# dglai/dgl-0.5-benchmark

Measured on AMD Instinct MI355X. Metric: aggregated edges/s, full-graph 3-layer GraphSAGE (hidden 64) on an ogbn-products-shaped graph; epoch time in ms_per_step, higher is better.
Workload: dtype f32

## Files before the change

dgl-0.5-benchmark_amd/csrc/xty.hip:

```cpp
#include "common.h"

namespace mgx {

constexpr int kXtyWaves = 2048;

static int xty_waves(int64_t n) {
  int64_t w = (n / 256 + 63) / 64 * 64;
  if (w < 256) w = 256;
  if (w > kXtyWaves) w = kXtyWaves;
  return (int)w;
}

template <int MT, int KT>
__global__ __launch_bounds__(kBlock) void xty_partial_kernel(int64_t n, int M, int K, const float* __restrict__ A, int64_t lda,
                                                             const float* __restrict__ B, int64_t ldb, float* __restrict__ part) {
  const int lane = threadIdx.x & (kWave - 1);
  const int64_t gw = (int64_t)blockIdx.x * kWavesPerBlock + threadIdx.x / kWave;
  const int c = lane % 16, q = lane / 16;
  v4f acc[MT][KT];
#pragma unroll
  for (int i = 0; i < MT; ++i)
#pragma unroll
    for (int j = 0; j < KT; ++j) acc[i][j] = (v4f)(0.f);
  bool am[MT], bm[KT];
#pragma unroll
  for (int i = 0; i < MT; ++i) am[i] = i * 16 + c < M;
#pragma unroll
// ... 6 lines not shown
      const int64_t row = r0 + s * 4 + q;
      const bool ok = row < n;
#pragma unroll
      for (int i = 0; i < MT; ++i) a[s][i] = (ok && am[i]) ? A[row * lda + i * 16 + c] : 0.f;
#pragma unroll
      for (int j = 0; j < KT; ++j) b[s][j] = (ok && bm[j]) ? B[row * ldb + j * 16 + c] : 0.f;
    }
#pragma unroll
    for (int s = 0; s < 4; ++s)
#pragma unroll
      for (int i = 0; i < MT; ++i)
#pragma unroll
        for (int j = 0; j < KT; ++j) acc[i][j] = __builtin_amdgcn_mfma_f32_16x16x4f32(a[s][i], b[s][j], acc[i][j], 0, 0, 0);
  }
  float* p = part + gw * (int64_t)(MT * 16) * (KT * 16);
#pragma unroll
  for (int i = 0; i < MT; ++i)
#pragma unroll
    for (int j = 0; j < KT; ++j)
#pragma unroll
      for (int r = 0; r < 4; ++r) p[(i * 16 + 4 * q + r) * (KT * 16) + j * 16 + c] = acc[i][j][r];
}

template <int AVG, int AST, int BVG, int BST>
__global__ __launch_bounds__(kBlock) void xty_partial_v4_kernel(int64_t n, int M, int K, int mt16, int kt16, const float* __restrict__ A,
                                                                int64_t lda, const float* __restrict__ B, int64_t ldb,
                                                                float* __restrict__ part, float* __restrict__ part_sum) {
  constexpr int AT = AVG * 4 + AST, BT = BVG * 4 + BST;
  const int lane = threadIdx.x & (kWave - 1);
  const int64_t gw = (int64_t)blockIdx.x * kWavesPerBlock + threadIdx.x / kWave;
  const int c = lane % 16, q = lane / 16;
  v4f acc[AT][BT];
  v4f accs[AT > 0 ? AT : 1];
#pragma unroll
  for (int i = 0; i < AT; ++i) {
    accs[i] = (v4f)(0.f);
#pragma unroll
    for (int j = 0; j < BT; ++j) acc[i][j] = (v4f)(0.f);
  }
  const float one = c == 0 ? 1.f : 0.f;
  const int64_t stride = (int64_t)gridDim.x * kWavesPerBlock * 16;
  for (int64_t r0 = gw * 16; r0 < n; r0 += stride) {
    float a[4][AT > 0 ? AT : 1], b[4][BT > 0 ? BT : 1];
#pragma unroll
    for (int s = 0; s < 4; ++s) {
      const int64_t row = r0 + s * 4 + q;
      const bool ok = row < n;
#pragma unroll
      for (int g = 0; g < AVG; ++g) {
        const v4f v = (ok && g * 64 + 4 * c + 3 < M) ? *reinterpret_cast<const v4f*>(A + row * lda + g * 64 + 4 * c) : (v4f)(0.f);
        a[s][g * 4 + 0] = v.x; a[s][g * 4 + 1] = v.y; a[s][g * 4 + 2] = v.z; a[s][g * 4 + 3] = v.w;
      }
#pragma unroll
      for (int i = 0; i < AST; ++i) a[s][AVG * 4 + i] = (ok && AVG * 64 + i * 16 + c < M) ? A[row * lda + AVG * 64 + i * 16 + c] : 0.f;
#pragma unroll
      for (int g = 0; g < BVG; ++g) {
        const v4f v = (ok && g * 64 + 4 * c + 3 < K) ? *reinterpret_cast<const v4f*>(B + row * ldb + g * 64 + 4 * c) : (v4f)(0.f);
        b[s][g * 4 + 0] = v.x; b[s][g * 4 + 1] = v.y; b[s][g * 4 + 2] = v.z; b[s][g * 4 + 3] = v.w;
      }
#pragma unroll
      for (int j = 0; j < BST; ++j) b[s][BVG * 4 + j] = (ok && BVG * 64 + j * 16 + c < K) ? B[row * ldb + BVG * 64 + j * 16 + c] : 0.f;
    }
#pragma unroll
    for (int s = 0; s < 4; ++s)
#pragma unroll
      for (int i = 0; i < AT; ++i)
#pragma unroll
        for (int j = 0; j < BT; ++j) acc[i][j] = __builtin_amdgcn_mfma_f32_16x16x4f32(a[s][i], b[s][j], acc[i][j], 0, 0, 0);
    if (part_sum) {
#pragma unroll
      for (int s = 0; s < 4; ++s)
#pragma unroll
        for (int i = 0; i < AT; ++i) accs[i] = __builtin_amdgcn_mfma_f32_16x16x4f32(a[s][i], (r0 + s * 4 + q < n) ? one : 0.f, accs[i], 0, 0, 0);
// ... 4 lines not shown
    for (int i = 0; i < AT; ++i)
#pragma unroll
      for (int r = 0; r < 4; ++r) {
        const int mi = 4 * q + r;
        const int m = i < AVG * 4 ? (i / 4) * 64 + 4 * mi + (i % 4) : AVG * 64 + (i - AVG * 4) * 16 + mi;
        if (m < mt16) part_sum[gw * (int64_t)mt16 + m] = accs[i][r];
      }
  }
  float* p = part + gw * (int64_t)mt16 * kt16;
#pragma unroll
  for (int i = 0; i < AT; ++i)
#pragma unroll
    for (int j = 0; j < BT; ++j) {
      const int k = j < BVG * 4 ? (j / 4) * 64 + 4 * c + (j % 4) : BVG * 64 + (j - BVG * 4) * 16 + c;
#pragma unroll
      for (int r = 0; r < 4; ++r) {
        const int mi = 4 * q + r;
        const int m = i < AVG * 4 ? (i / 4) * 64 + 4 * mi + (i % 4) : AVG * 64 + (i - AVG * 4) * 16 + mi;
        if (m < mt16 && k < kt16) p[m * kt16 + k] = acc[i][j][r];
      }
    }
}

template <int AVG, int AST>
static bool launch_xty_v4_b(int bvg, int bst, int waves, int64_t n, int M, int K, int mt16, int kt16, const float* A, int64_t lda,
                            const float* B, int64_t ldb, float* part, float* part_sum, hipStream_t s) {
#define MGX_XTY4(G, T) if (bvg == G && bst == T) { hipLaunchKernelGGL((xty_partial_v4_kernel<AVG, AST, G, T>), dim3(waves / kWavesPerBlock), dim3(kBlock), 0, s, n, M, K, mt16, kt16, A, lda, B, ldb, part, part_sum); return true; }
  MGX_XTY4(2, 0) MGX_XTY4(1, 0) MGX_XTY4(1, 1) MGX_XTY4(1, 2) MGX_XTY4(1, 3) MGX_XTY4(1, 4)
#undef MGX_XTY4
  return false;
}

static bool launch_xty_v4(int mt, int kt, int waves, int64_t n, int M, int K, const float* A, int64_t lda, const float* B, int64_t ldb,
                          float* part, float* part_sum, hipStream_t s) {
  const bool bvec = ldb % 4 == 0 && (uintptr_t)B % 16 == 0 && K % 4 == 0 && K >= 64;
  if (!bvec) return false;
  const int bvg = K >= 128 ? 2 : 1, bst = (K - bvg * 64 + 15) / 16;
  const bool avec = lda % 4 == 0 && (uintptr_t)A % 16 == 0 && M == 64;
  const int mt16 = mt * 16, kt16 = kt * 16;
  if (avec) return launch_xty_v4_b<1, 0>(bvg, bst, waves, n, M, K, mt16, kt16, A, lda, B, ldb, part, part_sum, s);
  switch (mt) {
    case 1: return launch_xty_v4_b<0, 1>(bvg, bst, waves, n, M, K, mt16, kt16, A, lda, B, ldb, part, part_sum, s);
    case 2: return launch_xty_v4_b<0, 2>(bvg, bst, waves, n, M, K, mt16, kt16, A, lda, B, ldb, part, part_sum, s);
    case 3: return launch_xty_v4_b<0, 3>(bvg, bst, waves, n, M, K, mt16, kt16, A, lda, B, ldb, part, part_sum, s);
    default: return launch_xty_v4_b<0, 4>(bvg, bst, waves, n, M, K, mt16, kt16, A, lda, B, ldb, part, part_sum, s);
  }
}

__global__ __launch_bounds__(kBlock) void xty_finish_kernel(int M, int K, int ldm , int tile , int waves,
                                                            const float* __restrict__ part, float* __restrict__ out, int64_t ldc) {
  __shared__ float red[16][17];
  const int e = threadIdx.x % 16, sl = threadIdx.x / 16;
  const int idx = blockIdx.x * 16 + e;
  float s0 = 0.f, s1 = 0.f, s2 = 0.f, s3 = 0.f;
  if (idx < M * K) {
    const int m = idx / K, k = idx % K;
    const float* p = part + (int64_t)m * ldm + k;
    const int per = waves / 16;
    for (int w = sl * per; w < (sl + 1) * per; w += 4) {
      s0 += p[(int64_t)w * tile];
      s1 += p[(int64_t)(w + 1) * tile];
      s2 += p[(int64_t)(w + 2) * tile];
      s3 += p[(int64_t)(w + 3) * tile];
    }
  }
  red[sl][e] = (s0 + s1) + (s2 + s3);
  __syncthreads();
  if (sl == 0 && idx < M * K) {
    float s = 0.f;
    for (int i = 0; i < 16; ++i) s += red[i][e];
    out[(int64_t)(idx / K) * ldc + idx % K] = s;
  }
}

constexpr int kXtyGridTotal = 4096;
constexpr int kXtyTileM = 64, kXtyTileK = 128;

__global__ __launch_bounds__(kBlock) void xty_partial_grid_kernel(int64_t n, int M, int K, int tiles_k, const float* __restrict__ A,
                                                                  int64_t lda, const float* __restrict__ B, int64_t ldb,
                                                                  float* __restrict__ part) {
  constexpr int MT = 4, KT = 8;
  const int tile = blockIdx.y;
  const int m0 = (tile / tiles_k) * kXtyTileM, k0 = (tile % tiles_k) * kXtyTileK;
  const int Mt = M - m0 < kXtyTileM ? M - m0 : kXtyTileM, Kt = K - k0 < kXtyTileK ? K - k0 : kXtyTileK;
  A += m0;
  B += k0;
  const int lane = threadIdx.x & (kWave - 1);
  const int64_t gw = (int64_t)blockIdx.x * kWavesPerBlock + threadIdx.x / kWave;
  const int c = lane % 16, q = lane / 16;
  v4f acc[MT][KT];
#pragma unroll
  for (int i = 0; i < MT; ++i)
#pragma unroll
    for (int j = 0; j < KT; ++j) acc[i][j] = (v4f)(0.f);
  bool am[MT], bm[KT];
#pragma unroll
  for (int i = 0; i < MT; ++i) am[i] = i * 16 + c < Mt;
#pragma unroll
  for (int j = 0; j < KT; ++j) bm[j] = j * 16 + c < Kt;
// ... 68 lines not shown
}

}

namespace mgx {
__global__ __launch_bounds__(kBlock) void xty_colsum_finish_kernel(int M, int mt16, int waves, const float* __restrict__ part_sum,
                                                                   float* __restrict__ colsum) {
  const int m = blockIdx.x * kWavesPerBlock + threadIdx.x / kWave;
  const int lane = threadIdx.x % kWave;
  if (m >= M) return;
  float s = 0.f;
  for (int w = lane; w < waves; w += kWave) s += part_sum[(int64_t)w * mt16 + m];
#pragma unroll
  for (int off = 32; off >= 1; off >>= 1) s += __shfl_xor(s, off, kWave);
  if (lane == 0) colsum[m] = s;
}
}

extern "C" int64_t mgx_xty_workspace(int64_t M, int64_t K) {
  const int64_t mt = (M + 15) / 16, kt = (K + 15) / 16;
  if (M < 1 || K < 1) return -1;
  if (mt > 4 || kt > 8) {
    if (M > 256 || K > 1024) return -1;
    return (int64_t)mgx::kXtyGridTotal * mgx::kXtyTileM * mgx::kXtyTileK * (int64_t)sizeof(float);
  }
  return (int64_t)mgx::kXtyWaves * (mt * 16 * kt * 16 + mt * 16) * (int64_t)sizeof(float);
}

static int32_t xty_impl(int64_t n, int64_t M, int64_t K, const float* a, int64_t lda, const float* b, int64_t ldb, float* out, int64_t ldc,
                        float* colsum, void* workspace, void* stream);

extern "C" int32_t mgx_xty(int64_t n, int64_t M, int64_t K, const float* a, int64_t lda, const float* b, int64_t ldb, float* out,
                           int64_t ldc, void* workspace, void* stream) {
  return xty_impl(n, M, K, a, lda, b, ldb, out, ldc, nullptr, workspace, stream);
}

extern "C" int32_t mgx_xty_colsum(int64_t n, int64_t M, int64_t K, const float* a, int64_t lda, const float* b, int64_t ldb, float* out,
                                  int64_t ldc, float* colsum, void* workspace, void* stream) {
  if (!colsum) return xty_impl(n, M, K, a, lda, b, ldb, out, ldc, nullptr, workspace, stream);
  return xty_impl(n, M, K, a, lda, b, ldb, out, ldc, colsum, workspace, stream);
}

static int32_t xty_impl(int64_t n, int64_t M, int64_t K, const float* a, int64_t lda, const float* b, int64_t ldb, float* out, int64_t ldc,
                        float* colsum, void* workspace, void* stream) {
  using namespace mgx;
  MGX_ENTER();
  MGX_CHECK_ARG(n >= 0 && M >= 1 && K >= 1, "mgx_xty: bad sizes");
  const int mt = (int)((M + 15) / 16), kt = (int)((K + 15) / 16);
  if (M > 256 || K > 1024) MGX_UNSUPPORTED("mgx_xty: needs M <= 256 and K <= 1024 (got %lld x %lld)", (long long)M, (long long)K);
  MGX_CHECK_ARG(out != nullptr, "mgx_xty: out is NULL");
  MGX_CHECK_ARG(lda >= M && ldb >= K && ldc >= K, "mgx_xty: leading dimensions smaller than the tile (lda %lld, ldb %lld, ldc %lld)",
                (long long)lda, (long long)ldb, (long long)ldc);
  hipStream_t s = (hipStream_t)stream;
  if (n == 0) {
    MGX_CHECK_HIP(hipMemset2DAsync(out, (size_t)ldc * sizeof(float), 0, (size_t)K * sizeof(float), (size_t)M, s));
    if (colsum) MGX_CHECK_HIP(hipMemsetAsync(colsum, 0, (size_t)M * sizeof(float), s));
    return MGX_OK;
  }
  MGX_CHECK_ARG(a && b && workspace, "mgx_xty: NULL pointer");
  float* part = (float*)workspace;
  if (mt > 4 || kt > 8) {
    if (colsum) MGX_UNSUPPORTED("mgx_xty_colsum: one 64 x 128 tile only");
    const int tiles_m = (int)((M + kXtyTileM - 1) / kXtyTileM), tiles_k = (int)((K + kXtyTileK - 1) / kXtyTileK);
    int wpt = kXtyGridTotal / (tiles_m * tiles_k) / 64 * 64;
    const int64_t by_rows = n / 128 / 64 * 64;
    if (wpt > by_rows) wpt = (int)by_rows;
    if (wpt < 64) wpt = 64;
    hipLaunchKernelGGL(xty_partial_grid_kernel, dim3(wpt / kWavesPerBlock, tiles_m * tiles_k), dim3(kBlock), 0, s, n, (int)M,
                       (int)K, tiles_k, a, lda, b, ldb, part);
    MGX_CHECK_LAUNCH();
    hipLaunchKernelGGL(xty_finish_grid_kernel, dim3(kXtyTileM * kXtyTileK / 16, tiles_m * tiles_k), dim3(kBlock), 0, s, (int)M, (int)K,
                       tiles_k, wpt, (const float*)part, out, ldc);
    MGX_CHECK_LAUNCH();
    return MGX_OK;
  }
  const int waves = xty_waves(n);
  float* part_sum = colsum ? part + (int64_t)kXtyWaves * mt * 16 * kt * 16 : nullptr;
  bool ok = launch_xty_v4(mt, kt, waves, n, (int)M, (int)K, a, lda, b, ldb, part, part_sum, s);
  if (!ok && colsum) MGX_UNSUPPORTED("mgx_xty_colsum: needs the 16-byte-load form (B: K %% 4 == 0, K >= 64, aligned)");
  if (!ok) switch (mt) {
    case 1: ok = launch_xty_kt<1>(kt, waves, n, (int)M, (int)K, a, lda, b, ldb, part, s); break;
    case 2: ok = launch_xty_kt<2>(kt, waves, n, (int)M, (int)K, a, lda, b, ldb, part, s); break;
    case 3: ok = launch_xty_kt<3>(kt, waves, n, (int)M, (int)K, a, lda, b, ldb, part, s); break;
    default: ok = launch_xty_kt<4>(kt, waves, n, (int)M, (int)K, a, lda, b, ldb, part, s); break;
  }
  MGX_CHECK_ARG(ok, "mgx_xty: no kernel for this tile shape");
  MGX_CHECK_LAUNCH();
  hipLaunchKernelGGL(xty_finish_kernel, dim3((unsigned)((M * K + 15) / 16)), dim3(kBlock), 0, s, (int)M, (int)K, kt * 16,
                     mt * 16 * kt * 16, waves, (const float*)part, out, ldc);
  MGX_CHECK_LAUNCH();
  if (colsum) {
    hipLaunchKernelGGL(xty_colsum_finish_kernel, dim3((unsigned)((M + kWavesPerBlock - 1) / kWavesPerBlock)), dim3(kBlock), 0, s, (int)M,
                       mt * 16, waves, (const float*)part_sum, colsum);
    MGX_CHECK_LAUNCH();
  }
  return MGX_OK;
}
```

dgl-0.5-benchmark_amd/mi355x_graph/_lib.py:

```python
import ctypes
import os

_HERE = os.path.dirname(os.path.abspath(__file__))
CSRC_DIR = os.path.normpath(os.path.join(_HERE, "..", "csrc"))
LIB_PATH = os.environ.get("MGX_LIB_PATH") or os.path.join(CSRC_DIR, "libmi355x_graph.so")
HEADER_PATH = os.path.normpath(os.path.join(_HERE, "..", "..", "include", "mi355x_graph.h"))


class DGLError(RuntimeError):
    """Error type of the DGL operator surface (re-exported as dgl.DGLError)."""


class MgxCsr(ctypes.Structure):
    _fields_ = [
        ("num_rows", ctypes.c_int64),
        ("num_cols", ctypes.c_int64),
        ("nnz", ctypes.c_int64),
        ("indptr", ctypes.c_void_p),
        ("indices", ctypes.c_void_p),
        ("eids", ctypes.c_void_p),
        ("idx_bits", ctypes.c_int32),
        ("reserved", ctypes.c_int32),
    ]

# ... 44 lines not shown
    "mgx_gat_fused_fwd": (_i32, [_csr_p, _vp, _i64, _i64, _fp, _fp, _fp, _fp, ctypes.c_float, ctypes.c_float, ctypes.c_uint64, _fp, _fp,
                                 _vp, _vp, _vp]),
    "mgx_gat_fused_bwd": (_i32, [_csr_p, _vp, _csr_p, _vp, _i64, _i64, _fp, _fp, _fp, ctypes.c_float, ctypes.c_float, ctypes.c_uint64,
                                 _fp, _fp, _fp, _fp, _fp, _fp, _vp, _vp, _vp]),
    "mgx_gat_tile_fwd": (_i32, [_csr_p, _vp, _vp, _i64, _i64, _fp, _fp, _fp, ctypes.c_float, ctypes.c_float, ctypes.c_uint64, _fp, _fp,
                                _vp, _vp, _vp]),
    "mgx_gat_tile_bwd": (_i32, [_csr_p, _vp, _vp, _csr_p, _vp, _vp, _i64, _i64, _fp, _fp, ctypes.c_float, ctypes.c_float, ctypes.c_uint64,
                                _fp, _fp, _fp, _fp, _fp, _fp, _vp, _vp, _vp]),
    "mgx_head_dot_fwd": (_i32, [_i64, _i64, _i64, _fp, _fp, _fp, _fp, _fp, _vp]),
    "mgx_head_dot_bwd_workspace": (_i64, [_i64, _i64]),
    "mgx_head_dot_bwd": (_i32, [_i64, _i64, _i64, _fp, _fp, _fp, _fp, _fp, _fp, _fp, _fp, _vp, _vp]),
    "mgx_segment_reduce": (_i32, [_i64, _vp, _i64, _i32, _fp, _fp, _vp, _vp]),
    "mgx_relu_dropout_fwd": (_i32, [_i64, _fp, ctypes.c_float, ctypes.c_uint64, ctypes.c_uint64, _fp, _vp, _vp]),
    "mgx_relu_dropout_bwd": (_i32, [_i64, _fp, _vp, ctypes.c_float, _fp, _vp]),
    "mgx_relu_dropout_fwd_strided": (_i32, [_i64, _i64, _fp, _i64, ctypes.c_float, ctypes.c_uint64, ctypes.c_uint64, _fp, _i64, _vp, _vp]),
    "mgx_relu_dropout_bwd_strided": (_i32, [_i64, _i64, _fp, _i64, _vp, ctypes.c_float, _fp, _i64, _vp]),
    "mgx_relu_dropout_bwd_slots": (_i32, [_i64, _fp, _i64, _vp, ctypes.c_float, _fp, _i64, _fp, _vp, _vp, _vp]),
    "mgx_relu_dropout_fwd_counter": (_i32, [_i64, _i64, _fp, _i64, ctypes.c_float, ctypes.c_uint64, _vp, _fp, _i64, _vp, _vp]),
    "mgx_column_pair_sums": (_i32, [_i64, _i64, _i32, _fp, _fp, _fp, _fp, _vp, _vp]),
    "mgx_column_affine": (_i32, [_i64, _i64, _fp, _fp, _fp, _fp, _fp, _fp, _vp]),
    "mgx_xty_workspace": (_i64, [_i64, _i64]),
    "mgx_xty": (_i32, [_i64, _i64, _i64, _fp, _i64, _fp, _i64, _fp, _i64, _vp, _vp]),
    "mgx_xty_colsum": (_i32, [_i64, _i64, _i64, _fp, _i64, _fp, _i64, _fp, _i64, _fp, _vp, _vp]),
    "mgx_rows_gemm": (_i32, [_i64, _i64, _i64, _fp, _i64, _fp, _i64, _i32, _fp, _fp, _i64, _fp, _i64, _fp, _i64, _i64, _vp]),
    "mgx_rows_gemm_supported": (_i32, [_i64, _i64, _i64]),
    "mgx_rows_gemm_relu_dropout": (_i32, [_i64, _i64, _i64, _fp, _i64, _fp, _i64, _i32, _fp, ctypes.c_float, ctypes.c_uint64, ctypes.c_uint64,
                                          _fp, _i64, _vp, _vp, _vp, _vp]),
    "mgx_column_sum_workspace": (_i64, [_i64]),
    "mgx_column_sum": (_i32, [_i64, _i64, _fp, _fp, _vp, _vp]),
    "mgx_coo_to_csr_workspace": (_i64, [_i64, _i64, _i32]),
    "mgx_coo_to_csr": (_i32, [_i64, _i64, _vp, _vp, _i32, _vp, _vp, _vp, _vp, _i64, _vp]),
    "mgx_csr_transpose_workspace": (_i64, [_i64, _i64, _i32]),
    "mgx_csr_transpose": (_i32, [_csr_p, _vp, _vp, _vp, _vp, _i64, _vp]),
    "mgx_csr_degrees": (_i32, [_i64, _vp, _i32, _vp, _vp]),
    "mgx_csr_inv_degrees": (_i32, [_i64, _vp, _i32, _fp, _vp]),
    "mgx_coo_to_csr_host": (_i32, [_i64, _i64, _vp, _vp, _i32, _vp, _vp, _vp]),
    "mgx_sample_neighbors": (_i32, [_csr_p, _i64, _vp, _i32, ctypes.c_uint64, _vp, _vp, _vp, _vp]),
    "mgx_gather_rows": (_i32, [_i64, _vp, _i32, _i64, _fp, _fp, _vp]),
    "mgx_gather_rows_strided": (_i32, [_i64, _vp, _i32, _i64, _fp, _i64, _fp, _i64, _vp]),
    "mgx_scatter_add_rows": (_i32, [_i64, _vp, _i32, _i64, _fp, _fp, _vp]),
}

_lib = None


def lib():
# ... 23 lines not shown
```

dgl-0.5-benchmark_amd/mi355x_graph/config.py:

```python

SAGE_FUSED_LAYER = True
SAGE_CAT = True
SAGE_STATIC_CAT = True
SAGE_FUSED_ADD = True
SAGE_FUSED_ACT = True
SAGE_PROJECT_FIRST = True
ROWS_GEMM = True
LINEAR_XTY = True
XTY_COLSUM = True

GAT_AGG_FIRST = True
GAT_PACK = True

PLAN_BUILDER = "device"
HUB_SPLIT = 256
LP_ROUNDS = 8
CLUSTER_MIN_NNZ = 4_000_000
TILE_HUB_SPLIT = 2048
TILE_CONFIG = {4: (7, 6, 1, 3), 3: (7, 3, 1, 3), 2: (7, 3, 1, 2)}
GAT_TILE_CONFIG = (7, 3, 1, 2)
TILE_MIN_WIDTH = 4
TILE_VALIDATE = True
SHORT_ROWS_IMBALANCE = 6.0

SPARSE_GRAD = False
SPARSE_GRAD_MIN_NNZ = 2_000_000
WIDE_PAD = True
WIDE_PAD_MIN_NNZ = 1 << 20

PACKED_GATHER = True
PACKED_GATHER_MIN_NNZ = 20_000_000
PACKED_GATHER_PROBE = True
# ... 5 lines not shown
```

dgl-0.5-benchmark_amd/mi355x_graph/ops.py:

```python
import os

import torch
from torch.autograd.function import once_differentiable

from ._lib import DGLError
from . import sparse
from . import config
from .graph import DGLGraph, GraphIndex

__all__ = ["gspmm", "rel_gspmm", "gsddmm", "edge_softmax", "gat_attention", "gat_fused", "segment_reduce", "copy_u_sum", "copy_u_mean", "u_mul_e_sum",
           "copy_e_sum", "u_add_v", "u_dot_v"]


def _torch_ops():
    if os.environ.get("MGX_TORCH_OPS", "auto") != "1":
        return None
    from . import torch_ops
    return torch_ops


_NATIVE = None


def _native_ops():
# ... 634 lines not shown


def batch_norm_supported(x):
    return (x.dim() == 2 and x.dtype == torch.float32 and x.device.type in sparse._BACKENDS and x.shape[1] % 4 == 0
            and 4 <= x.shape[1] <= sparse.backend_for(x).COLUMN_SUM_MAX and x.shape[0] > 1)


def _weight_grad(dy2, x2):
    be = sparse.backend_for(dy2)
    if (x2.shape[0] >= be.XTY_MIN_ROWS and dy2.shape[1] <= be.XTY_MAX[0] and x2.shape[1] <= be.XTY_MAX[1]
            and config.LINEAR_XTY):
        return be.xty(dy2 if dy2.stride(1) == 1 else dy2.contiguous(), x2 if x2.stride(1) == 1 else x2.contiguous())
    return dy2.t() @ x2


def _weight_bias_grad(dy2, x2):
    be = sparse.backend_for(dy2)
    if (x2.shape[0] >= be.XTY_MIN_ROWS and dy2.shape[1] <= be.XTY_MAX[0] and x2.shape[1] <= be.XTY_MAX[1]
            and config.LINEAR_XTY and config.XTY_COLSUM):
        return be.xty(dy2 if dy2.stride(1) == 1 else dy2.contiguous(), x2 if x2.stride(1) == 1 else x2.contiguous(), colsum=True)
    return _weight_grad(dy2, x2), be.column_sum(dy2 if dy2.is_contiguous() else dy2.contiguous())


class LinearSumFn(torch.autograd.Function):

    @staticmethod
    def forward(ctx, x1, w1, x2, w2, bias):
        ctx.save_for_backward(x1, w1, x2, w2)
        y = torch.nn.functional.linear(x1, w1, bias)
        return y.addmm_(x2, w2.t())

    @staticmethod
    @once_differentiable
    def backward(ctx, dy):
        x1, w1, x2, w2 = ctx.saved_tensors
        dy = dy.contiguous()
        need = ctx.needs_input_grad
        dx1 = dy @ w1 if need[0] else None
        dw1 = _weight_grad(dy, x1) if need[1] else None
        dx2 = dy @ w2 if need[2] else None
        dw2 = _weight_grad(dy, x2) if need[3] else None
        db = sparse.backend_for(dy).column_sum(dy) if need[4] else None
        return dx1, dw1, dx2, dw2, db


def linear_sum(x1, weight1, x2, weight2, bias=None):
# ... 134 lines not shown
                y, mask = be.relu_dropout_fwd(_rows_linear(be, cat.buf, wcat, bias), float(p), seed, offset,
                                              out=None if into is None else into.t)
            else:
                y, mask = fused
            ctx.save_for_backward(w_self, w_neigh, mask)
            ctx.p = float(p)
            return y
        ctx.save_for_backward(w_self, w_neigh)
        ctx.p = None
        return _rows_linear(be, cat.buf, torch.cat([w_self, w_neigh], dim=1), bias)

    @staticmethod
    @once_differentiable
    def backward(ctx, dy):
        cat = ctx.cat
        if cat.generation != ctx.generation:
            raise DGLError("SAGEConv: a later forward pass overwrote the [h | neigh] buffer this backward pass needs "
                           "(two forwards before one backward); set MGX_SAGE_CAT=0")
        need = ctx.needs_input_grad
        be = sparse.backend_for(dy)
        K = cat.K
        dh = None
        aggregated_first = False
        if ctx.p is not None:
            w_self, w_neigh, mask = ctx.saved_tensors
            if not dy.is_contiguous() and not be._row_strided(dy):
                dy = dy.contiguous()
            gate = None
            if need[2] and dy.dim() == 2 and dy.shape[1] == 64 and K % 4 == 0 and config.ROWS_GEMM and be.rows_gemm_supported(128, K, 128):
                gate = _slot_gate(be, ctx.gidx, ctx.gidx.csr(), dy.shape[0])
                if gate is not None and not gate.allow():
                    gate = None
            if gate is not None:
                dcat = torch.empty((dy.shape[0], 128), dtype=torch.float32, device=dy.device)
                inv = ctx.gidx.csc().inv_degrees()
                if dy.data_ptr() % 16 == 0:
                    dy, slots, overflow = be.relu_dropout_bwd_slots(dy, mask, ctx.p, dcat[:, :64], row_scale=inv)
                else:
                    dy = be.relu_dropout_bwd(dy, mask, ctx.p, out=dcat[:, :64])
                    slots, overflow = be.rows_slots_pack(dy, row_scale=inv)
                gate.watch(overflow, dy.shape[0])
                be.spmm_copy_u_strided(ctx.gidx.csr(), "sum", dy, dcat[:, 64:], slots=slots, src_scale=inv)
                dh = be.rows_gemm(dcat, torch.cat([w_self, w_neigh], dim=0))
                if dh is None:
                    dh = dcat @ torch.cat([w_self, w_neigh], dim=0)
                aggregated_first = True
            else:
                dy = be.relu_dropout_bwd(dy, mask, ctx.p)
        else:
            w_self, w_neigh = ctx.saved_tensors
        if not aggregated_first:
            dy = dy.contiguous()
        if need[2] and not aggregated_first:
            dh, dn = _rows_dgrad(be, dy, torch.cat([w_self, w_neigh], dim=1), ctx.gidx.csc().inv_degrees(), K)
            be.spmm_copy_u_strided(ctx.gidx.csr(), "sum", dn, dh, accumulate=True)
        dws = dwn = db = None
        if (need[3] or need[4]) and need[5]:
            dw, db = _weight_bias_grad(dy, cat.buf)
            dws, dwn = dw[:, :K].contiguous(), dw[:, K:].contiguous()
        elif need[3] or need[4]:
            dw = _weight_grad(dy, cat.buf)
            dws, dwn = dw[:, :K].contiguous(), dw[:, K:].contiguous()
        elif need[5]:
            db = be.column_sum(dy if dy.is_contiguous() else dy.contiguous())
        return None, None, dh, dws, dwn, db, None


_ROW_BITS = {}


def _row_bits(rows, n, be):
    key = (rows.data_ptr(), int(rows.shape[0]), int(n))
    held = _ROW_BITS.get(key)
    if held is None or held[0] is not rows:
        flag = torch.zeros((n, 4), dtype=torch.float32, device=rows.device)
        flag[rows] = 1.0
        if len(_ROW_BITS) > 8:
            _ROW_BITS.clear()
        held = _ROW_BITS[key] = (rows, be.row_nonzero_bits(flag))
    return held[1]
# ... 459 lines not shown
```

dgl-0.5-benchmark_amd/mi355x_graph/sparse.py:

```python
import ctypes
import os
import functools

import numpy as np
import torch

from . import _lib
from ._lib import DGLError, MgxCsr, OP, REDUCE, TARGET
from . import config


PROFILE = None


class timed_call(object):
    __slots__ = ("rec", "dev")

    def __init__(self, dev, **meta):
        self.rec, self.dev = (meta if PROFILE is not None else None), dev

    def __enter__(self):
        if self.rec is not None:
            self.rec["start"] = torch.cuda.Event(enable_timing=True)
            self.rec["end"] = torch.cuda.Event(enable_timing=True)
# ... 902 lines not shown
        n, M = a2d.shape
        K = b2d.shape[1]
        if M > self.XTY_MAX[0] or K > self.XTY_MAX[1]:
            raise DGLError("mgx_xty: at most %d x %d outputs, got %d x %d" % (self.XTY_MAX + (M, K)))
        out = torch.empty((M, K), dtype=torch.float32, device=dev)
        sums = torch.empty(M, dtype=torch.float32, device=dev) if colsum else None
        have_sums = False
        L = _lib.lib()
        tm, tk = self.XTY_TILE
        ntiles = ((M + tm - 1) // tm) * ((K + tk - 1) // tk)

        def one(a_t, b_t, o_t, ws, want_sums):
            if want_sums:
                st = L.mgx_xty_colsum(n, a_t.shape[1], b_t.shape[1], _ptr(a_t), max(a2d.stride(0), M), _ptr(b_t), max(b2d.stride(0), K),
                                      _ptr(o_t), out.stride(0), _ptr(sums), _ptr(ws), _stream(dev))
                if st != _lib.ERR_UNSUPPORTED:
                    _lib.check(st)
                    return True
            _lib.check(L.mgx_xty(n, a_t.shape[1], b_t.shape[1], _ptr(a_t), max(a2d.stride(0), M), _ptr(b_t), max(b2d.stride(0), K),
                                 _ptr(o_t), out.stride(0), _ptr(ws), _stream(dev)))
            return False

        with torch.cuda.device(dev):
            if ntiles == 1 or ntiles >= 4:
                ws = torch.empty(max(L.mgx_xty_workspace(M, K), 4) // 4, dtype=torch.float32, device=dev)
                have_sums = one(a2d, b2d, out, ws, colsum and ntiles == 1)
            else:
                ws = torch.empty(max(L.mgx_xty_workspace(min(M, tm), min(K, tk)), 4) // 4, dtype=torch.float32, device=dev)
                for m0 in range(0, M, tm):
                    for k0 in range(0, K, tk):
                        a_t, b_t, o_t = a2d[:, m0:m0 + tm], b2d[:, k0:k0 + tk], out[m0:m0 + tm, k0:k0 + tk]
                        if one(a_t, b_t, o_t, ws, colsum and M <= tm and k0 == 0):
                            have_sums = True
        if not colsum:
            return out
        return out, (sums if have_sums else self.column_sum(a2d if a2d.is_contiguous() else a2d.contiguous()))

    def rows_gemm(self, a2d, b2d, b_transposed=False, bias=None, row_scale=None, scale_from=0, out=None, split_col=0):
        dev = self._check_dev(a2d, b2d, bias, row_scale, out)
        n, K = a2d.shape
        M = b2d.shape[0] if b_transposed else b2d.shape[1]
        if (a2d.stride(1) != 1 or b2d.stride(1) != 1 or (b2d.shape[1] if b_transposed else b2d.shape[0]) != K
                or a2d.dtype != torch.float32 or b2d.dtype != torch.float32):
            return None
        out2 = None
        if split_col:
            out = torch.empty((n, split_col), dtype=torch.float32, device=dev)
            out2 = torch.empty((n, M - split_col), dtype=torch.float32, device=dev)
        elif out is None:
            out = torch.empty((n, M), dtype=torch.float32, device=dev)
        with torch.cuda.device(dev):
            st = _lib.lib().mgx_rows_gemm(n, K, M, _ptr(a2d), a2d.stride(0), _ptr(b2d), b2d.stride(0), 1 if b_transposed else 0,
                                          _ptr(bias), _ptr(row_scale), int(scale_from), _ptr(out), out.stride(0), _ptr(out2),
                                          0 if out2 is None else out2.stride(0), int(split_col), _stream(dev))
        if st == _lib.ERR_UNSUPPORTED:
            return None
        _lib.check(st)
        return out if out2 is None else (out, out2)

# ... 302 lines not shown
```

include/mi355x_graph.h:

```cpp
#ifndef MI355X_GRAPH_H_
#define MI355X_GRAPH_H_

#include <stdint.h>

#ifdef __cplusplus
extern "C" {
#endif

typedef enum {
  MGX_OK = 0,
  MGX_ERR_INVALID_ARGUMENT = 1,
  MGX_ERR_UNSUPPORTED = 2,
  MGX_ERR_HIP = 3
} mgx_status;

typedef enum {
  MGX_OP_ADD = 0, MGX_OP_SUB = 1, MGX_OP_MUL = 2, MGX_OP_DIV = 3,
  MGX_OP_COPY_LHS = 4, MGX_OP_COPY_RHS = 5, MGX_OP_DOT = 6
} mgx_op;

typedef enum { MGX_REDUCE_SUM = 0, MGX_REDUCE_MAX = 1, MGX_REDUCE_MIN = 2, MGX_REDUCE_MEAN = 3 } mgx_reduce;

enum {
  MGX_SPMM_ACCUMULATE = 1,
// ... 155 lines not shown
int32_t mgx_head_dot_fwd(int64_t n, int64_t H, int64_t F, const float* feat, const float* attn_a,
                         const float* attn_b, float* out_a, float* out_b, void* stream);
int64_t mgx_head_dot_bwd_workspace(int64_t H, int64_t F);
int32_t mgx_head_dot_bwd(int64_t n, int64_t H, int64_t F, const float* feat, const float* attn_a,
                         const float* attn_b, const float* d_out_a, const float* d_out_b, float* d_feat,
                         float* d_attn_a, float* d_attn_b, void* workspace, void* stream);

int32_t mgx_segment_reduce(int64_t num_segments, const int64_t* offsets, int64_t D, int32_t reduce,
                           const float* x, float* out, int64_t* arg, void* stream);

int64_t mgx_column_sum_workspace(int64_t C);
int32_t mgx_column_sum(int64_t n, int64_t C, const float* x, float* out, void* workspace, void* stream);

int32_t mgx_column_pair_sums(int64_t n, int64_t C, int32_t mode, const float* a, const float* b, float* out0, float* out1,
                             void* workspace, void* stream);
int32_t mgx_column_affine(int64_t n, int64_t C, const float* a, const float* b, const float* A, const float* B, const float* Cc,
                          float* out, void* stream);

int64_t mgx_xty_workspace(int64_t M, int64_t K);
int32_t mgx_xty(int64_t n, int64_t M, int64_t K, const float* a, int64_t lda, const float* b, int64_t ldb, float* out, int64_t ldc,
                void* workspace, void* stream);
int32_t mgx_xty_colsum(int64_t n, int64_t M, int64_t K, const float* a, int64_t lda, const float* b, int64_t ldb, float* out, int64_t ldc,
                       float* colsum, void* workspace, void* stream);

int32_t mgx_rows_gemm(int64_t n, int64_t K, int64_t M, const float* a, int64_t lda, const float* b, int64_t ldb, int32_t b_transposed,
                      const float* bias , const float* row_scale , int64_t scale_from, float* c,
                      int64_t ldc, float* c2 ,
                      int64_t ldc2, int64_t split_col , void* stream);
int32_t mgx_rows_gemm_supported(int64_t K, int64_t M, int64_t lda);
int32_t mgx_rows_gemm_relu_dropout(int64_t n, int64_t K, int64_t M, const float* a, int64_t lda, const float* b, int64_t ldb,
                                   int32_t b_transposed, const float* bias , float p, uint64_t seed, uint64_t offset,
                                   float* y, int64_t ldy, uint8_t* mask, void* slots ,
                                   int64_t* overflow_rows , void* stream);

int32_t mgx_relu_dropout_fwd(int64_t n, const float* x, float p, uint64_t seed, uint64_t offset, float* y, uint8_t* mask,
                             void* stream);
int32_t mgx_relu_dropout_bwd(int64_t n, const float* dy, const uint8_t* mask, float p, float* dx, void* stream);
int32_t mgx_relu_dropout_fwd_strided(int64_t rows, int64_t cols, const float* x, int64_t x_stride, float p, uint64_t seed,
                                     uint64_t offset, float* y, int64_t y_stride, uint8_t* mask, void* stream);
int32_t mgx_relu_dropout_bwd_strided(int64_t rows, int64_t cols, const float* dy, int64_t dy_stride, const uint8_t* mask, float p,
                                     float* dx, int64_t dx_stride, void* stream);
int32_t mgx_relu_dropout_bwd_slots(int64_t rows, const float* dy, int64_t dy_stride, const uint8_t* mask, float p, float* dx,
                                   int64_t dx_stride, const float* row_scale , void* slots ,
                                   int64_t* overflow_rows , void* stream);
int32_t mgx_relu_dropout_fwd_counter(int64_t rows, int64_t cols, const float* x, int64_t x_stride, float p, uint64_t seed,
                                     const uint64_t* counter, float* y, int64_t y_stride, uint8_t* mask, void* stream);
// ... 41 lines not shown
```

Measured before the change: 37.93 billion.

## Fuse relu-dropout backward mask into XtY weight-grad and add two-tile split kernel

Adds a masked XtY path that applies the saved relu-dropout mask and 1/(1-p) scale while loading dy, so the weight and bias gradients for the first SAGE layer no longer need a separate relu_dropout_bwd pass and a materialized dy. It also adds a split kernel for M=64, K in 192..256 that runs two K tiles (128 plus the remainder) inside one launch, interleaved across XCDs, with a finish kernel that reads both partial buffers. This replaces the generic grid path for that shape and lets colsum be produced from the same pass. The cost is a larger workspace and more template instantiations, and the fused path only runs when the input gradient is not needed.

```diff
diff --git a/dgl-0.5-benchmark_amd/csrc/xty.hip b/dgl-0.5-benchmark_amd/csrc/xty.hip
--- a/dgl-0.5-benchmark_amd/csrc/xty.hip
+++ b/dgl-0.5-benchmark_amd/csrc/xty.hip
@@ -3,6 +3,7 @@
 namespace mgx {
 
 constexpr int kXtyWaves = 2048;
+constexpr int kXtyTileM = 64, kXtyTileK = 128;
 
 static int xty_waves(int64_t n) {
   int64_t w = (n / 256 + 63) / 64 * 64;
@@ -55,13 +56,14 @@
       for (int r = 0; r < 4; ++r) p[(i * 16 + 4 * q + r) * (KT * 16) + j * 16 + c] = acc[i][j][r];
 }
 
-template <int AVG, int AST, int BVG, int BST>
-__global__ __launch_bounds__(kBlock) void xty_partial_v4_kernel(int64_t n, int M, int K, int mt16, int kt16, const float* __restrict__ A,
-                                                                int64_t lda, const float* __restrict__ B, int64_t ldb,
-                                                                float* __restrict__ part, float* __restrict__ part_sum) {
+template <int AVG, int AST, int BVG, int BST, bool MASKED>
+__device__ __forceinline__ void xty_partial_v4_body(int64_t n, int M, int K, int mt16, int kt16, const float* __restrict__ A, int64_t lda,
+                                                    const float* __restrict__ B, int64_t ldb, float* __restrict__ part,
+                                                    float* __restrict__ part_sum, const uint8_t* __restrict__ mask, float scale,
+                                                    int64_t gw, int64_t nwaves) {
+  static_assert(!MASKED || (AVG == 1 && AST == 0), "the mask is 4 bits per float4 of a 64-column row");
   constexpr int AT = AVG * 4 + AST, BT = BVG * 4 + BST;
   const int lane = threadIdx.x & (kWave - 1);
-  const int64_t gw = (int64_t)blockIdx.x * kWavesPerBlock + threadIdx.x / kWave;
   const int c = lane % 16, q = lane / 16;
   v4f acc[AT][BT];
   v4f accs[AT > 0 ? AT : 1];
@@ -72,7 +74,7 @@
     for (int j = 0; j < BT; ++j) acc[i][j] = (v4f)(0.f);
   }
   const float one = c == 0 ? 1.f : 0.f;
-  const int64_t stride = (int64_t)gridDim.x * kWavesPerBlock * 16;
+  const int64_t stride = nwaves * 16;
   for (int64_t r0 = gw * 16; r0 < n; r0 += stride) {
     float a[4][AT > 0 ? AT : 1], b[4][BT > 0 ? BT : 1];
 #pragma unroll
@@ -81,7 +83,14 @@
       const bool ok = row < n;
 #pragma unroll
       for (int g = 0; g < AVG; ++g) {
-        const v4f v = (ok && g * 64 + 4 * c + 3 < M) ? *reinterpret_cast<const v4f*>(A + row * lda + g * 64 + 4 * c) : (v4f)(0.f);
+        v4f v = (ok && g * 64 + 4 * c + 3 < M) ? *reinterpret_cast<const v4f*>(A + row * lda + g * 64 + 4 * c) : (v4f)(0.f);
+        if (MASKED) {
+          const uint8_t m = ok ? mask[row * 16 + c] : (uint8_t)0;
+          v.x = (m & 1) ? v.x * scale : 0.f;
+          v.y = (m & 2) ? v.y * scale : 0.f;
+          v.z = (m & 4) ? v.z * scale : 0.f;
+          v.w = (m & 8) ? v.w * scale : 0.f;
+        }
         a[s][g * 4 + 0] = v.x; a[s][g * 4 + 1] = v.y; a[s][g * 4 + 2] = v.z; a[s][g * 4 + 3] = v.w;
       }
 #pragma unroll
@@ -132,33 +141,77 @@
     }
 }
 
-template <int AVG, int AST>
+template <int AVG, int AST, int BVG, int BST, bool MASKED>
+__global__ __launch_bounds__(kBlock) void xty_partial_v4_kernel(int64_t n, int M, int K, int mt16, int kt16, const float* __restrict__ A,
+                                                                int64_t lda, const float* __restrict__ B, int64_t ldb,
+                                                                float* __restrict__ part, float* __restrict__ part_sum,
+                                                                const uint8_t* __restrict__ mask, float scale) {
+  xty_partial_v4_body<AVG, AST, BVG, BST, MASKED>(n, M, K, mt16, kt16, A, lda, B, ldb, part, part_sum, mask, scale,
+                                                  (int64_t)blockIdx.x * kWavesPerBlock + threadIdx.x / kWave,
+                                                  (int64_t)gridDim.x * kWavesPerBlock);
+}
+
+template <int BVG2, int BST2, bool MASKED>
+__global__ __launch_bounds__(kBlock) void xty_partial_split_kernel(int64_t n, int M, int K, int mt16, int kt16b, const float* __restrict__ A,
+                                                                   int64_t lda, const float* __restrict__ B, int64_t ldb,
+                                                                   float* __restrict__ part, float* __restrict__ part_b,
+                                                                   float* __restrict__ part_sum, const uint8_t* __restrict__ mask,
+                                                                   float scale) {
+  const int b = blockIdx.x;
+  const int64_t gw = (int64_t)((b >> 4) * kXcds + (b & (kXcds - 1))) * kWavesPerBlock + threadIdx.x / kWave;
+  const int64_t nwaves = (int64_t)(gridDim.x / 2) * kWavesPerBlock;
+  if (((b >> 3) & 1) == 0)
+    xty_partial_v4_body<1, 0, 2, 0, MASKED>(n, M, kXtyTileK, mt16, kXtyTileK, A, lda, B, ldb, part, part_sum, mask, scale, gw, nwaves);
+  else
+    xty_partial_v4_body<1, 0, BVG2, BST2, MASKED>(n, M, K - kXtyTileK, mt16, kt16b, A, lda, B + kXtyTileK, ldb, part_b, nullptr, mask, scale,
+                                                  gw, nwaves);
+}
+
+template <int AVG, int AST, bool MASKED>
 static bool launch_xty_v4_b(int bvg, int bst, int waves, int64_t n, int M, int K, int mt16, int kt16, const float* A, int64_t lda,
-                            const float* B, int64_t ldb, float* part, float* part_sum, hipStream_t s) {
-#define MGX_XTY4(G, T) if (bvg == G && bst == T) { hipLaunchKernelGGL((xty_partial_v4_kernel<AVG, AST, G, T>), dim3(waves / kWavesPerBlock), dim3(kBlock), 0, s, n, M, K, mt16, kt16, A, lda, B, ldb, part, part_sum); return true; }
+                            const float* B, int64_t ldb, float* part, float* part_sum, const uint8_t* mask, float scale, hipStream_t s) {
+#define MGX_XTY4(G, T) if (bvg == G && bst == T) { hipLaunchKernelGGL((xty_partial_v4_kernel<AVG, AST, G, T, MASKED>), dim3(waves / kWavesPerBlock), dim3(kBlock), 0, s, n, M, K, mt16, kt16, A, lda, B, ldb, part, part_sum, mask, scale); return true; }
   MGX_XTY4(2, 0) MGX_XTY4(1, 0) MGX_XTY4(1, 1) MGX_XTY4(1, 2) MGX_XTY4(1, 3) MGX_XTY4(1, 4)
 #undef MGX_XTY4
   return false;
 }
 
+static bool xty_vec_operand(const float* p, int64_t ld) { return ld % 4 == 0 && (uintptr_t)p % 16 == 0; }
+
 static bool launch_xty_v4(int mt, int kt, int waves, int64_t n, int M, int K, const float* A, int64_t lda, const float* B, int64_t ldb,
-                          float* part, float* part_sum, hipStream_t s) {
-  const bool bvec = ldb % 4 == 0 && (uintptr_t)B % 16 == 0 && K % 4 == 0 && K >= 64;
+                          float* part, float* part_sum, const uint8_t* mask, float scale, hipStream_t s) {
+  const bool bvec = xty_vec_operand(B, ldb) && K % 4 == 0 && K >= 64;
   if (!bvec) return false;
   const int bvg = K >= 128 ? 2 : 1, bst = (K - bvg * 64 + 15) / 16;
-  const bool avec = lda % 4 == 0 && (uintptr_t)A % 16 == 0 && M == 64;
+  const bool avec = xty_vec_operand(A, lda) && M == 64;
   const int mt16 = mt * 16, kt16 = kt * 16;
-  if (avec) return launch_xty_v4_b<1, 0>(bvg, bst, waves, n, M, K, mt16, kt16, A, lda, B, ldb, part, part_sum, s);
+  if (mask) return avec && launch_xty_v4_b<1, 0, true>(bvg, bst, waves, n, M, K, mt16, kt16, A, lda, B, ldb, part, part_sum, mask, scale, s);
+  if (avec) return launch_xty_v4_b<1, 0, false>(bvg, bst, waves, n, M, K, mt16, kt16, A, lda, B, ldb, part, part_sum, mask, scale, s);
   switch (mt) {
-    case 1: return launch_xty_v4_b<0, 1>(bvg, bst, waves, n, M, K, mt16, kt16, A, lda, B, ldb, part, part_sum, s);
-    case 2: return launch_xty_v4_b<0, 2>(bvg, bst, waves, n, M, K, mt16, kt16, A, lda, B, ldb, part, part_sum, s);
-    case 3: return launch_xty_v4_b<0, 3>(bvg, bst, waves, n, M, K, mt16, kt16, A, lda, B, ldb, part, part_sum, s);
-    default: return launch_xty_v4_b<0, 4>(bvg, bst, waves, n, M, K, mt16, kt16, A, lda, B, ldb, part, part_sum, s);
-  }
+    case 1: return launch_xty_v4_b<0, 1, false>(bvg, bst, waves, n, M, K, mt16, kt16, A, lda, B, ldb, part, part_sum, mask, scale, s);
+    case 2: return launch_xty_v4_b<0, 2, false>(bvg, bst, waves, n, M, K, mt16, kt16, A, lda, B, ldb, part, part_sum, mask, scale, s);
+    case 3: return launch_xty_v4_b<0, 3, false>(bvg, bst, waves, n, M, K, mt16, kt16, A, lda, B, ldb, part, part_sum, mask, scale, s);
+    default: return launch_xty_v4_b<0, 4, false>(bvg, bst, waves, n, M, K, mt16, kt16, A, lda, B, ldb, part, part_sum, mask, scale, s);
+  }
+}
+
+static bool xty_split_applies(int64_t M, int64_t K, const float* A, int64_t lda, const float* B, int64_t ldb) {
+  return M == kXtyTileM && K >= kXtyTileK + 64 && K <= 2 * kXtyTileK && K % 4 == 0 && xty_vec_operand(A, lda) && xty_vec_operand(B, ldb);
+}
+
+template <bool MASKED>
+static bool launch_xty_split(int waves, int64_t n, int M, int K, const float* A, int64_t lda, const float* B, int64_t ldb, float* part,
+                             float* part_b, float* part_sum, const uint8_t* mask, float scale, hipStream_t s) {
+  const int K2 = K - kXtyTileK, bvg = K2 >= 128 ? 2 : 1, bst = (K2 - bvg * 64 + 15) / 16, kt16b = (K2 + 15) / 16 * 16;
+#define MGX_XTYS(G, T) if (bvg == G && bst == T) { hipLaunchKernelGGL((xty_partial_split_kernel<G, T, MASKED>), dim3(2 * waves / kWavesPerBlock), dim3(kBlock), 0, s, n, M, K, kXtyTileM, kt16b, A, lda, B, ldb, part, part_b, part_sum, mask, scale); return true; }
+  MGX_XTYS(2, 0) MGX_XTYS(1, 0) MGX_XTYS(1, 1) MGX_XTYS(1, 2) MGX_XTYS(1, 3) MGX_XTYS(1, 4)
+#undef MGX_XTYS
+  return false;
 }
 
 __global__ __launch_bounds__(kBlock) void xty_finish_kernel(int M, int K, int ldm , int tile , int waves,
-                                                            const float* __restrict__ part, float* __restrict__ out, int64_t ldc) {
+                                                            const float* __restrict__ part, float* __restrict__ out, int64_t ldc, int ksplit,
+                                                            int ldm_b, int tile_b, const float* __restrict__ part_b) {
   __shared__ float red[16][17];
   const int e = threadIdx.x % 16, sl = threadIdx.x / 16;
   const int idx = blockIdx.x * 16 + e;
@@ -166,6 +219,10 @@
   if (idx < M * K) {
     const int m = idx / K, k = idx % K;
     const float* p = part + (int64_t)m * ldm + k;
+    if (k >= ksplit) {
+      p = part_b + (int64_t)m * ldm_b + (k - ksplit);
+      tile = tile_b;
+    }
     const int per = waves / 16;
     for (int w = sl * per; w < (sl + 1) * per; w += 4) {
       s0 += p[(int64_t)w * tile];
@@ -184,7 +241,6 @@
 }
 
 constexpr int kXtyGridTotal = 4096;
-constexpr int kXtyTileM = 64, kXtyTileK = 128;
 
 __global__ __launch_bounds__(kBlock) void xty_partial_grid_kernel(int64_t n, int M, int K, int tiles_k, const float* __restrict__ A,
                                                                   int64_t lda, const float* __restrict__ B, int64_t ldb,
@@ -299,27 +355,37 @@
   if (M < 1 || K < 1) return -1;
   if (mt > 4 || kt > 8) {
     if (M > 256 || K > 1024) return -1;
-    return (int64_t)mgx::kXtyGridTotal * mgx::kXtyTileM * mgx::kXtyTileK * (int64_t)sizeof(float);
+    int64_t floats = (int64_t)mgx::kXtyGridTotal * mgx::kXtyTileM * mgx::kXtyTileK;
+    if (M == mgx::kXtyTileM && K <= 2 * mgx::kXtyTileK)
+      floats = (int64_t)mgx::kXtyWaves * (2 * mgx::kXtyTileM * mgx::kXtyTileK + mgx::kXtyTileM);
+    return floats * (int64_t)sizeof(float);
   }
   return (int64_t)mgx::kXtyWaves * (mt * 16 * kt * 16 + mt * 16) * (int64_t)sizeof(float);
 }
 
-static int32_t xty_impl(int64_t n, int64_t M, int64_t K, const float* a, int64_t lda, const float* b, int64_t ldb, float* out, int64_t ldc,
-                        float* colsum, void* workspace, void* stream);
+static int32_t xty_impl(int64_t n, int64_t M, int64_t K, const float* a, int64_t lda, const uint8_t* mask, float p, const float* b,
+                        int64_t ldb, float* out, int64_t ldc, float* colsum, void* workspace, void* stream);
 
 extern "C" int32_t mgx_xty(int64_t n, int64_t M, int64_t K, const float* a, int64_t lda, const float* b, int64_t ldb, float* out,
                            int64_t ldc, void* workspace, void* stream) {
-  return xty_impl(n, M, K, a, lda, b, ldb, out, ldc, nullptr, workspace, stream);
+  return xty_impl(n, M, K, a, lda, nullptr, 0.f, b, ldb, out, ldc, nullptr, workspace, stream);
 }
 
 extern "C" int32_t mgx_xty_colsum(int64_t n, int64_t M, int64_t K, const float* a, int64_t lda, const float* b, int64_t ldb, float* out,
                                   int64_t ldc, float* colsum, void* workspace, void* stream) {
-  if (!colsum) return xty_impl(n, M, K, a, lda, b, ldb, out, ldc, nullptr, workspace, stream);
-  return xty_impl(n, M, K, a, lda, b, ldb, out, ldc, colsum, workspace, stream);
-}
-
-static int32_t xty_impl(int64_t n, int64_t M, int64_t K, const float* a, int64_t lda, const float* b, int64_t ldb, float* out, int64_t ldc,
-                        float* colsum, void* workspace, void* stream) {
+  return xty_impl(n, M, K, a, lda, nullptr, 0.f, b, ldb, out, ldc, colsum, workspace, stream);
+}
+
+extern "C" int32_t mgx_xty_colsum_masked(int64_t n, int64_t M, int64_t K, const float* a, int64_t lda, const uint8_t* mask, float p,
+                                         const float* b, int64_t ldb, float* out, int64_t ldc, float* colsum, void* workspace,
+                                         void* stream) {
+  MGX_CHECK_ARG(p >= 0.f && p < 1.f, "mgx_xty_colsum_masked: p must be in [0, 1)");
+  MGX_CHECK_ARG(mask != nullptr || n == 0, "mgx_xty_colsum_masked: mask is NULL");
+  return xty_impl(n, M, K, a, lda, mask, p, b, ldb, out, ldc, colsum, workspace, stream);
+}
+
+static int32_t xty_impl(int64_t n, int64_t M, int64_t K, const float* a, int64_t lda, const uint8_t* mask, float p, const float* b,
+                        int64_t ldb, float* out, int64_t ldc, float* colsum, void* workspace, void* stream) {
   using namespace mgx;
   MGX_ENTER();
   MGX_CHECK_ARG(n >= 0 && M >= 1 && K >= 1, "mgx_xty: bad sizes");
@@ -328,6 +394,8 @@
   MGX_CHECK_ARG(out != nullptr, "mgx_xty: out is NULL");
   MGX_CHECK_ARG(lda >= M && ldb >= K && ldc >= K, "mgx_xty: leading dimensions smaller than the tile (lda %lld, ldb %lld, ldc %lld)",
                 (long long)lda, (long long)ldb, (long long)ldc);
+  if (mask && !(M == kXtyTileM && xty_vec_operand(a, lda)))
+    MGX_UNSUPPORTED("mgx_xty_colsum_masked: a must have 64 columns, a row stride that is a multiple of 4 and a 16-byte aligned pointer");
   hipStream_t s = (hipStream_t)stream;
   if (n == 0) {
     MGX_CHECK_HIP(hipMemset2DAsync(out, (size_t)ldc * sizeof(float), 0, (size_t)K * sizeof(float), (size_t)M, s));
@@ -336,7 +404,27 @@
   }
   MGX_CHECK_ARG(a && b && workspace, "mgx_xty: NULL pointer");
   float* part = (float*)workspace;
+  const float scale = 1.f / (1.f - p);
+  if ((mt > 4 || kt > 8) && xty_split_applies(M, K, a, lda, b, ldb)) {
+    const int waves = xty_waves(n), kt16b = kt * 16 - kXtyTileK;
+    float* part_b = part + (int64_t)kXtyWaves * kXtyTileM * kXtyTileK;
+    float* part_sum = colsum ? part_b + (int64_t)kXtyWaves * kXtyTileM * kXtyTileK : nullptr;
+    const bool ok = mask ? launch_xty_split<true>(waves, n, (int)M, (int)K, a, lda, b, ldb, part, part_b, part_sum, mask, scale, s)
+                         : launch_xty_split<false>(waves, n, (int)M, (int)K, a, lda, b, ldb, part, part_b, part_sum, mask, scale, s);
+    MGX_CHECK_ARG(ok, "mgx_xty: no kernel for this tile shape");
+    MGX_CHECK_LAUNCH();
+    hipLaunchKernelGGL(xty_finish_kernel, dim3((unsigned)((M * K + 15) / 16)), dim3(kBlock), 0, s, (int)M, (int)K, kXtyTileK,
+                       kXtyTileM * kXtyTileK, waves, (const float*)part, out, ldc, kXtyTileK, kt16b, kXtyTileM * kt16b, (const float*)part_b);
+    MGX_CHECK_LAUNCH();
+    if (colsum) {
+      hipLaunchKernelGGL(xty_colsum_finish_kernel, dim3((unsigned)((M + kWavesPerBlock - 1) / kWavesPerBlock)), dim3(kBlock), 0, s, (int)M,
+                         kXtyTileM, waves, (const float*)part_sum, colsum);
+      MGX_CHECK_LAUNCH();
+    }
+    return MGX_OK;
+  }
   if (mt > 4 || kt > 8) {
+    if (mask) MGX_UNSUPPORTED("mgx_xty_colsum_masked: one 64 x 128 tile, or 64 x 192 .. 256 with 16-byte loads");
     if (colsum) MGX_UNSUPPORTED("mgx_xty_colsum: one 64 x 128 tile only");
     const int tiles_m = (int)((M + kXtyTileM - 1) / kXtyTileM), tiles_k = (int)((K + kXtyTileK - 1) / kXtyTileK);
     int wpt = kXtyGridTotal / (tiles_m * tiles_k) / 64 * 64;
@@ -353,7 +441,8 @@
   }
   const int waves = xty_waves(n);
   float* part_sum = colsum ? part + (int64_t)kXtyWaves * mt * 16 * kt * 16 : nullptr;
-  bool ok = launch_xty_v4(mt, kt, waves, n, (int)M, (int)K, a, lda, b, ldb, part, part_sum, s);
+  bool ok = launch_xty_v4(mt, kt, waves, n, (int)M, (int)K, a, lda, b, ldb, part, part_sum, mask, scale, s);
+  if (!ok && mask) MGX_UNSUPPORTED("mgx_xty_colsum_masked: needs the 16-byte-load form (B: K %% 4 == 0, K >= 64, aligned)");
   if (!ok && colsum) MGX_UNSUPPORTED("mgx_xty_colsum: needs the 16-byte-load form (B: K %% 4 == 0, K >= 64, aligned)");
   if (!ok) switch (mt) {
     case 1: ok = launch_xty_kt<1>(kt, waves, n, (int)M, (int)K, a, lda, b, ldb, part, s); break;
@@ -364,7 +453,7 @@
   MGX_CHECK_ARG(ok, "mgx_xty: no kernel for this tile shape");
   MGX_CHECK_LAUNCH();
   hipLaunchKernelGGL(xty_finish_kernel, dim3((unsigned)((M * K + 15) / 16)), dim3(kBlock), 0, s, (int)M, (int)K, kt * 16,
-                     mt * 16 * kt * 16, waves, (const float*)part, out, ldc);
+                     mt * 16 * kt * 16, waves, (const float*)part, out, ldc, (int)K, 0, 0, (const float*)nullptr);
   MGX_CHECK_LAUNCH();
   if (colsum) {
     hipLaunchKernelGGL(xty_colsum_finish_kernel, dim3((unsigned)((M + kWavesPerBlock - 1) / kWavesPerBlock)), dim3(kBlock), 0, s, (int)M,
diff --git a/dgl-0.5-benchmark_amd/mi355x_graph/_lib.py b/dgl-0.5-benchmark_amd/mi355x_graph/_lib.py
--- a/dgl-0.5-benchmark_amd/mi355x_graph/_lib.py
+++ b/dgl-0.5-benchmark_amd/mi355x_graph/_lib.py
@@ -90,6 +90,7 @@
     "mgx_xty_workspace": (_i64, [_i64, _i64]),
     "mgx_xty": (_i32, [_i64, _i64, _i64, _fp, _i64, _fp, _i64, _fp, _i64, _vp, _vp]),
     "mgx_xty_colsum": (_i32, [_i64, _i64, _i64, _fp, _i64, _fp, _i64, _fp, _i64, _fp, _vp, _vp]),
+    "mgx_xty_colsum_masked": (_i32, [_i64, _i64, _i64, _fp, _i64, _vp, ctypes.c_float, _fp, _i64, _fp, _i64, _fp, _vp, _vp]),
     "mgx_rows_gemm": (_i32, [_i64, _i64, _i64, _fp, _i64, _fp, _i64, _i32, _fp, _fp, _i64, _fp, _i64, _fp, _i64, _i64, _vp]),
     "mgx_rows_gemm_supported": (_i32, [_i64, _i64, _i64]),
     "mgx_rows_gemm_relu_dropout": (_i32, [_i64, _i64, _i64, _fp, _i64, _fp, _i64, _i32, _fp, ctypes.c_float, ctypes.c_uint64, ctypes.c_uint64,
diff --git a/dgl-0.5-benchmark_amd/mi355x_graph/config.py b/dgl-0.5-benchmark_amd/mi355x_graph/config.py
--- a/dgl-0.5-benchmark_amd/mi355x_graph/config.py
+++ b/dgl-0.5-benchmark_amd/mi355x_graph/config.py
@@ -8,6 +8,7 @@
 ROWS_GEMM = True
 LINEAR_XTY = True
 XTY_COLSUM = True
+XTY_MASKED = True
 
 GAT_AGG_FIRST = True
 GAT_PACK = True
diff --git a/dgl-0.5-benchmark_amd/mi355x_graph/ops.py b/dgl-0.5-benchmark_amd/mi355x_graph/ops.py
--- a/dgl-0.5-benchmark_amd/mi355x_graph/ops.py
+++ b/dgl-0.5-benchmark_amd/mi355x_graph/ops.py
@@ -680,6 +680,13 @@
     return _weight_grad(dy2, x2), be.column_sum(dy2 if dy2.is_contiguous() else dy2.contiguous())
 
 
+def _masked_weight_bias_grad(be, dy2, mask, p, x2, want_db):
+    if not (config.XTY_MASKED and config.LINEAR_XTY and config.XTY_COLSUM and hasattr(be, "xty_masked") and not capture_path()
+            and dy2.dim() == 2 and x2.shape[0] >= be.XTY_MIN_ROWS and dy2.shape[1] <= be.XTY_MAX[0] and x2.shape[1] <= be.XTY_MAX[1]):
+        return None
+    return be.xty_masked(dy2, mask, p, x2, colsum=want_db)
+
+
 class LinearSumFn(torch.autograd.Function):
 
     @staticmethod
@@ -860,6 +867,7 @@
         K = cat.K
         dh = None
         aggregated_first = False
+        masked = None
         if ctx.p is not None:
             w_self, w_neigh, mask = ctx.saved_tensors
             if not dy.is_contiguous() and not be._row_strided(dy):
@@ -884,16 +892,22 @@
                     dh = dcat @ torch.cat([w_self, w_neigh], dim=0)
                 aggregated_first = True
             else:
-                dy = be.relu_dropout_bwd(dy, mask, ctx.p)
+                if not need[2] and (need[3] or need[4]):
+                    masked = _masked_weight_bias_grad(be, dy, mask, ctx.p, cat.buf, need[5])
+                if masked is None:
+                    dy = be.relu_dropout_bwd(dy, mask, ctx.p)
         else:
             w_self, w_neigh = ctx.saved_tensors
-        if not aggregated_first:
+        if not aggregated_first and masked is None:
             dy = dy.contiguous()
         if need[2] and not aggregated_first:
             dh, dn = _rows_dgrad(be, dy, torch.cat([w_self, w_neigh], dim=1), ctx.gidx.csc().inv_degrees(), K)
             be.spmm_copy_u_strided(ctx.gidx.csr(), "sum", dn, dh, accumulate=True)
         dws = dwn = db = None
-        if (need[3] or need[4]) and need[5]:
+        if masked is not None:
+            dw, db = masked
+            dws, dwn = dw[:, :K].contiguous(), dw[:, K:].contiguous()
+        elif (need[3] or need[4]) and need[5]:
             dw, db = _weight_bias_grad(dy, cat.buf)
             dws, dwn = dw[:, :K].contiguous(), dw[:, K:].contiguous()
         elif need[3] or need[4]:
diff --git a/dgl-0.5-benchmark_amd/mi355x_graph/sparse.py b/dgl-0.5-benchmark_amd/mi355x_graph/sparse.py
--- a/dgl-0.5-benchmark_amd/mi355x_graph/sparse.py
+++ b/dgl-0.5-benchmark_amd/mi355x_graph/sparse.py
@@ -948,9 +948,9 @@
             return False
 
         with torch.cuda.device(dev):
-            if ntiles == 1 or ntiles >= 4:
+            if ntiles == 1 or ntiles >= 4 or self._xty_two_tiles(a2d, b2d):
                 ws = torch.empty(max(L.mgx_xty_workspace(M, K), 4) // 4, dtype=torch.float32, device=dev)
-                have_sums = one(a2d, b2d, out, ws, colsum and ntiles == 1)
+                have_sums = one(a2d, b2d, out, ws, colsum and ntiles <= 2)
             else:
                 ws = torch.empty(max(L.mgx_xty_workspace(min(M, tm), min(K, tk)), 4) // 4, dtype=torch.float32, device=dev)
                 for m0 in range(0, M, tm):
@@ -961,6 +961,31 @@
         if not colsum:
             return out
         return out, (sums if have_sums else self.column_sum(a2d if a2d.is_contiguous() else a2d.contiguous()))
+
+    @staticmethod
+    def _xty_two_tiles(a2d, b2d):
+        K = b2d.shape[1]
+        return (a2d.shape[1] == 64 and 192 <= K <= 256 and K % 4 == 0 and a2d.stride(0) % 4 == 0 and b2d.stride(0) % 4 == 0
+                and a2d.data_ptr() % 16 == 0 and b2d.data_ptr() % 16 == 0)
+
+    def xty_masked(self, a2d, mask, p, b2d, colsum=True):
+        dev = self._check_dev(a2d, b2d, mask)
+        n, M = a2d.shape
+        K = b2d.shape[1]
+        L = _lib.lib()
+        nbytes = L.mgx_xty_workspace(M, K)
+        if nbytes < 0 or a2d.stride(1) != 1 or b2d.stride(1) != 1 or mask.numel() * 4 != n * M:
+            return None
+        out = torch.empty((M, K), dtype=torch.float32, device=dev)
+        sums = torch.empty(M, dtype=torch.float32, device=dev) if colsum else None
+        ws = torch.empty(max(nbytes, 4) // 4, dtype=torch.float32, device=dev)
+        with torch.cuda.device(dev):
+            st = L.mgx_xty_colsum_masked(n, M, K, _ptr(a2d), max(a2d.stride(0), M), _ptr(mask), ctypes.c_float(p), _ptr(b2d),
+                                         max(b2d.stride(0), K), _ptr(out), out.stride(0), _ptr(sums), _ptr(ws), _stream(dev))
+        if st == _lib.ERR_UNSUPPORTED:
+            return None
+        _lib.check(st)
+        return out, sums
 
     def rows_gemm(self, a2d, b2d, b_transposed=False, bias=None, row_scale=None, scale_from=0, out=None, split_col=0):
         dev = self._check_dev(a2d, b2d, bias, row_scale, out)
diff --git a/include/mi355x_graph.h b/include/mi355x_graph.h
--- a/include/mi355x_graph.h
+++ b/include/mi355x_graph.h
@@ -201,6 +201,8 @@
                 void* workspace, void* stream);
 int32_t mgx_xty_colsum(int64_t n, int64_t M, int64_t K, const float* a, int64_t lda, const float* b, int64_t ldb, float* out, int64_t ldc,
                        float* colsum, void* workspace, void* stream);
+int32_t mgx_xty_colsum_masked(int64_t n, int64_t M, int64_t K, const float* a, int64_t lda, const uint8_t* mask, float p, const float* b,
+                              int64_t ldb, float* out, int64_t ldc, float* colsum, void* workspace, void* stream);
 
 int32_t mgx_rows_gemm(int64_t n, int64_t K, int64_t M, const float* a, int64_t lda, const float* b, int64_t ldb, int32_t b_transposed,
                       const float* bias , const float* row_scale , int64_t scale_from, float* c,
```

After: 37.91 billion, median of 3. No clear change (-0.1%).
